# ucsdarclab/Python-SuPer

Measured on AMD Instinct MI355X. Metric: LM iterations/s (embedded-deformation LM, point-to-plane + ARAP + Rot), higher is better.
Workload: dtype f64

## Files before the change

### python-super_amd/csrc/slm_api.hip

```cpp
#include <atomic>
#include <condition_variable>
#include <functional>
#include <mutex>
#include <new>
#include <string>
#include <thread>
#include <algorithm>
#include <vector>
#include <cstdio>
#include <cstring>

#include "slm_common.h"
#include "slm_host.h"
#include "slm_launch.h"
#include "slm_prep.h"

static thread_local std::string g_err;
static const char* const kBadKnn =
    "slm_bind_frame: a KNN index (sf_knn_idx or ed_knn_idx) lies outside [0, J) or a surfel's row of sf_knn_idx repeats an id";

void slm_set_error_text(const char* msg) { g_err = msg; }

namespace {
template <typename T>
struct PinnedBuf {
  T* p = nullptr;
  size_t cap = 0, n = 0;
  hipError_t resize(size_t need) {
    if (need > cap) {
      if (p) (void)hipHostFree(p);
      p = nullptr;
      cap = 0;
      const size_t want = need + need / 8 + 16;
      const hipError_t e = hipHostMalloc((void**)&p, want * sizeof(T), hipHostMallocDefault);
      if (e != hipSuccess) return e;
      cap = want;
    }
    n = need;
    return hipSuccess;
  }
  void release() {
    if (p) (void)hipHostFree(p);
    p = nullptr;
    cap = n = 0;
  }
  T* data() { return p; }
  const T* data() const { return p; }
  size_t size() const { return n; }
  T* begin() { return p; }
  T* end() { return p + n; }
  T& operator[](size_t i) { return p[i]; }
  const T& operator[](size_t i) const { return p[i]; }
};

constexpr int kLossBlocks = 512;
constexpr int kRegBlocksMax = 64;

enum class DataForm {
  none,
  tuple,
  pairs,
  per_entry,
};
DataForm data_form_of(const slm_config& c, const slm_frame& f) {
  if (!c.use_data || f.N <= 0) return DataForm::none;
// ... 146 lines not shown

 private:
  void ensure(int n_workers) {
    while ((int)threads_.size() < n_workers) {
      const int id = (int)threads_.size();
      threads_.emplace_back([this, id] { loop(id); });
    }
  }
  void loop(int id) {
    int seen = 0;
    for (;;) {
      const std::function<void(int)>* job = nullptr;
      {
        std::unique_lock<std::mutex> lk(m_);
        cv_work_.wait(lk, [&] { return stop_ || generation_ != seen; });
        if (stop_) return;
        seen = generation_;
        if (id < n_active_) job = job_;
      }
      if (job) {
        (*job)(id + 1);
        std::lock_guard<std::mutex> lk(m_);
        if (--pending_ == 0) cv_done_.notify_all();
      }
    }
  }
  std::vector<std::thread> threads_;
  std::mutex m_;
  std::condition_variable cv_work_, cv_done_;
  const std::function<void(int)>* job_ = nullptr;
  int generation_ = 0, n_active_ = 0, pending_ = 0;
  bool stop_ = false;
};
}

struct slm_solver {
  PrepBuffers* prep = nullptr;
  BindPool bind_pool;
  AsyncWorker prep_worker;
  PrepBuffers* prep_async = nullptr;
  hipStream_t prep_stream = nullptr;
  std::vector<PrepBuffers*> bind_prep;
  std::vector<hipStream_t> bind_streams;
  std::vector<hipEvent_t> bind_events;
  std::mutex band_mutex;
  hipEvent_t drain_event = nullptr;
  double drain_est_ms = 0.0;
  int last_solver_form = -1;
  int last_dag_mode = -1;
  bool no_reuse = false;
  bool hybrid_batches = true;
  long dag_max_nodes = 8000;
  bool fuse_begin = true;
  bool pure_fill = true;
  bool profile = false;
  std::vector<hipEvent_t> ev_pool;
  std::vector<std::vector<hipEvent_t>> ev_runs;
  slm_config cfg{};
  std::vector<Slot> slots;
  FrameDev* frames_dev = nullptr;
  int* bw_dev = nullptr;
  int* bw_host = nullptr;
  int* reuse_dev = nullptr;
  int rank = 0, world = 1;
  bool shard_mode = false;
};
namespace {
bool solve_is_task_graph(const slm_solver* s, int n, int J);
}

static std::atomic<long long> g_reallocs{0}, g_realloc_bytes{0}, g_plan_builds{0}, g_plan_reuses{0}, g_plan_fill_hits{0};

template <typename T>
static hipError_t grow(T*& p, size_t& cap, size_t need) {
  if (need <= cap) return hipSuccess;
  const size_t want = need + need / 8;
  ++g_reallocs;
  g_realloc_bytes += (long long)(want * sizeof(T));
  return grow(p, cap, need, want);
}
template <typename T>
static hipError_t grow(GP<T>& p, size_t& cap, size_t need) {
  T* q = p;
  const hipError_t e = grow(q, cap, need);
  p = q;
  return e;
}

static int check_slots(slm_solver* s, int first, int n);

extern "C" {

const char* slm_last_error(void) { return g_err.c_str(); }

int slm_debug_last_solver_form(slm_solver* s) { return s ? s->last_solver_form : -1; }
int slm_debug_last_dag_mode(slm_solver* s) { return s ? s->last_dag_mode : -1; }

int slm_debug_counters(int64_t out[4]) {
  if (!out) return fail(SLM_ERR_INVALID, "slm_debug_counters: null output");
  out[0] = g_reallocs;
  out[1] = g_realloc_bytes;
  out[2] = g_plan_builds;
  out[3] = g_plan_reuses;
  return SLM_OK;
}

// ... 103 lines not shown
             sizeof(slm_frame), sizeof(slm_gf_config), sizeof(slm_gf_frame), sizeof(slm_iter_record));
    return fail(SLM_ERR_INVALID, buf);
  }
  return SLM_OK;
}

int slm_device_count(void) {
  int n = 0;
  if (hipGetDeviceCount(&n) != hipSuccess) return 0;
  return n;
}

int slm_create(const slm_config* cfg, slm_solver** out) {
  if (!cfg || !out) return fail(SLM_ERR_INVALID, "slm_create: null argument");
  if (cfg->max_frames < 1 || cfg->num_iterations < 0 || !(cfg->v > 0.0))
    return fail(SLM_ERR_INVALID, "slm_create: bad config");
  if (cfg->solver_path < 0 || cfg->solver_path > 4) return fail(SLM_ERR_INVALID, "slm_create: solver_path must be 0..4");
  if (cfg->data_path < 0 || cfg->data_path > 2) return fail(SLM_ERR_INVALID, "slm_create: data_path must be 0..2");
  if (slm_device_count() < 1) return fail(SLM_ERR_NO_DEVICE, "slm_create: no HIP device visible");
  slm_solver* s = new (std::nothrow) slm_solver();
  if (!s) return fail(SLM_ERR_HIP, "slm_create: out of host memory");
  s->cfg = *cfg;
  try {
    s->slots.resize(cfg->max_frames);
  } catch (...) {
    delete s;
    return fail(SLM_ERR_HIP, "slm_create: out of host memory");
  }
  hipError_t e = hipMalloc((void**)&s->frames_dev, sizeof(FrameDev) * cfg->max_frames);
  if (e == hipSuccess) e = hipMemset(s->frames_dev, 0, sizeof(FrameDev) * cfg->max_frames);
  if (e == hipSuccess) e = hipMalloc((void**)&s->bw_dev, 2 * sizeof(int));
  if (e == hipSuccess) e = hipMalloc((void**)&s->reuse_dev, sizeof(int) * cfg->max_frames);
  if (e == hipSuccess) e = hipMemset(s->reuse_dev, 0, sizeof(int) * cfg->max_frames);
  if (e == hipSuccess) e = hipHostMalloc((void**)&s->bw_host, 2 * sizeof(int), hipHostMallocDefault);
  if (e == hipSuccess) {
    s->prep = prep_create();
    if (!s->prep) e = hipErrorOutOfMemory;
  }
  if (e != hipSuccess) {
    g_err = std::string("slm_create: ") + hipGetErrorString(e);
    slm_destroy(s);
    return SLM_ERR_HIP;
  }
  {
    int dev = 0;
    (void)hipGetDevice(&dev);
    (void)dag_device_setup(dev, nullptr);
  }
  if (const char* hb = getenv("SLM_HYBRID")) s->hybrid_batches = atoi(hb) != 0;
  if (const char* dm = getenv("SLM_DAG_MAX_NODES")) s->dag_max_nodes = atol(dm);
  if (const char* nr = getenv("SLM_NO_REUSE")) s->no_reuse = atoi(nr) != 0;
  if (const char* pf = getenv("SLM_PURE_FILL")) s->pure_fill = atoi(pf) != 0;
  if (const char* fb = getenv("SLM_FUSE_BEGIN")) s->fuse_begin = atoi(fb) != 0;
  *out = s;
  return SLM_OK;
}

int slm_destroy(slm_solver* s) {
  if (!s) return SLM_OK;
  s->prep_worker.shutdown();
  s->bind_pool.shutdown();
  for (Slot& sl : s->slots) {
    FrameDev& h = sl.h;
    if (h.beta) (void)hipFree(h.beta);
    if (h.delta) (void)hipFree(h.delta);
    if (h.rhs) (void)hipFree(h.rhs);
    if (sl.band) (void)hipFree(sl.band);
    if (sl.linv) (void)hipFree(sl.linv);
    if (h.loss_part) (void)hipFree(h.loss_part);
    if (h.st) (void)hipFree(h.st);
    if (h.rec) (void)hipFree(h.rec);
    if (h.node_pk) (void)hipFree(h.node_pk);
    if (h.tgt_pn) (void)hipFree(h.tgt_pn);
    if (h.tgt_px) (void)hipFree(h.tgt_px);
    if (h.ev_rc) (void)hipFree(h.ev_rc);
    plan_free(sl.plan);
    pairplan_free(sl.pplan);
    if (sl.h_pin) (void)hipHostFree(sl.h_pin);
    sl.h_pairs.release();
    sl.h_knn.release();
    sl.h_pts.release();
    sl.h_pts64.release();
    if (sl.d_fronts) (void)hipFree(sl.d_fronts);
    if (sl.d_items) (void)hipFree(sl.d_items);
    if (sl.d_tile_kind) (void)hipFree(sl.d_tile_kind);
    if (sl.d_zero_tiles) (void)hipFree(sl.d_zero_tiles);
    if (sl.d_ints) (void)hipFree(sl.d_ints);
    if (sl.d_dests) (void)hipFree(sl.d_dests);
    if (sl.d_cur_dests) (void)hipFree(sl.d_cur_dests);
    if (sl.ftiles) (void)hipFree(sl.ftiles);
    if (sl.fvec) (void)hipFree(sl.fvec);
    if (sl.flinv) (void)hipFree(sl.flinv);
    if (sl.fmail) (void)hipFree(sl.fmail);
    if (sl.pairbuf) (void)hipFree(sl.pairbuf);
    if (sl.d_dag_flags) (void)hipFree(sl.d_dag_flags);
    if (sl.d_dag_trace) (void)hipFree(sl.d_dag_trace);
    if (sl.prep_fork) (void)hipEventDestroy(sl.prep_fork);
    if (sl.prep_done) (void)hipEventDestroy(sl.prep_done);
  }
  prep_destroy(s->prep);
  prep_destroy(s->prep_async);
  if (s->prep_stream) (void)hipStreamDestroy(s->prep_stream);
  for (PrepBuffers* pb : s->bind_prep) prep_destroy(pb);
  for (hipStream_t q : s->bind_streams) (void)hipStreamDestroy(q);
  for (hipEvent_t e : s->bind_events) (void)hipEventDestroy(e);
  for (auto& evs : s->ev_runs)
// ... 599 lines not shown
        if (rc != SLM_OK) {
          rcs[w] = rc;
          errs[w] = g_err;
          return;
        }
      }
      if (hipEventRecord(s->bind_events[w], s->bind_streams[w]) != hipSuccess) rcs[w] = SLM_ERR_HIP;
    } catch (...) {
      rcs[w] = SLM_ERR_HIP;
      try { errs[w] = "slm_bind_frames: out of host memory in a bind worker"; } catch (...) {}
    }
  };
  try {
    s->bind_pool.run(W, work);
  } catch (...) {
    return fail(SLM_ERR_HIP, "slm_bind_frames: could not start the bind workers");
  }
  for (int w = 0; w < W; ++w)
    if (rcs[w] != SLM_OK) return fail(rcs[w], errs[w].c_str());
  if (bind_trace_threshold() >= 0.0 && bt_now() - bt1 > bind_trace_threshold())
    fprintf(stderr, "[slm bind trace] batch of %d: drained the stream at %.3f (waited %.3f ms), workers done %.3f ms later\n",
            n_frames, bt1, bt1 - bt0, bt_now() - bt1);
  for (int w = 0; w < W; ++w) HIPCHK(hipStreamWaitEvent(st, s->bind_events[w], 0));
  return SLM_OK;
}

}

static int check_slots(slm_solver* s, int first, int n) {
  if (!s) return fail(SLM_ERR_INVALID, "null solver");
  if (first < 0 || n < 1 || first + n > (int)s->slots.size())
    return fail(SLM_ERR_INVALID, "slot range out of bounds");
  for (int i = first; i < first + n; ++i) {
    join_prepare(s, i);
    if (!s->slots[i].h.bound) return fail(SLM_ERR_UNBOUND, "slot used before slm_bind_frame");
    if (s->slots[i].h.f.K != s->slots[first].h.f.K)
      return fail(SLM_ERR_UNSUPPORTED, "the frames of one batch must have the same num_neighbors");
  }
  return SLM_OK;
}

namespace {
struct BatchDims {
  int maxN = 0, maxJKe = 0, nt_max = 0, wb_cap = 0, n_reg_part = 0;
  int max_pos = 0, max_blocks = 0, maxP = 0;
  int K = 0;
  int gram_variants = 0;
  bool nd = true;
  DataForm form = DataForm::none;
  const int* reuse = nullptr;
  bool fused_begin = false;
  int* accept_reuse = nullptr;
  int accept_eval = 0;
  int max_tasks = 0;
  int hybrid_cut = -2, hybrid_levels = -1, max_top_tasks = 0;
  std::vector<NDLevelSched> sched;
};
BatchDims dims_of(slm_solver* s, int first, int n, bool band = false) {
  BatchDims d;
  bool all_v1 = true, all_vk = true;
  for (int i = first; i < first + n; ++i) {
    const FrameDev& h = s->slots[i].h;
    d.maxN = std::max(d.maxN, h.f.N);
    d.K = (d.K == 0 || d.K == h.f.K) ? h.f.K : -1;
    d.maxJKe = std::max(d.maxJKe, h.f.J * h.f.K_ED);
    d.nt_max = std::max(d.nt_max, h.nt);
    d.wb_cap = std::max(d.wb_cap, h.wb);
    d.max_pos = std::max(d.max_pos, h.n_pos);
    d.max_blocks = std::max(d.max_blocks, h.n_blocks);
    all_v1 = all_v1 && h.v1_ready;
    all_vk = all_vk && h.vk_ready;
    if (h.v1_ready) d.gram_variants |= h.v2_ready ? 1 : 2;
    d.nd = d.nd && h.nd_ready;
    d.max_tasks = std::max(d.max_tasks, h.nd_ready ? h.n_dag_tasks : 0);
    if (h.nd_ready) {
      const int cut = h.n_dag_top_tasks > 0 ? h.dag_cut_depth : -1;
      if (d.hybrid_cut == -2) { d.hybrid_cut = cut; d.hybrid_levels = h.n_levels; }
      else if (d.hybrid_cut != cut || d.hybrid_levels != h.n_levels) d.hybrid_cut = -1;
      d.max_top_tasks = std::max(d.max_top_tasks, h.n_dag_top_tasks);
    }
    d.maxP = std::max(d.maxP, h.P);
  }
  d.nd = d.nd && !band;
  const slm_config& c = s->cfg;
  d.form = all_v1 ? DataForm::tuple : (d.nd && all_vk) ? DataForm::pairs : c.use_data ? DataForm::per_entry : DataForm::none;
  const bool tuple = d.form == DataForm::tuple;
  if (d.nd && tuple && c.phase_test && !s->no_reuse) d.reuse = s->reuse_dev + first;
  d.fused_begin = d.nd && tuple && d.gram_variants == 1 && d.max_pos > 0 && s->fuse_begin;
  if (tuple && c.phase_test) d.accept_reuse = s->reuse_dev + first;
  d.accept_eval = tuple ? 1 : 0;
  if (d.nd) {
    for (int i = first; i < first + n; ++i) {
      const auto& sc = s->slots[i].cache.nd.sched;
      if (sc.size() > d.sched.size()) d.sched.resize(sc.size(), NDLevelSched{0, 0, 0, 0, 0, -2, 0, -2, 0, -2});
      for (size_t l = 0; l < sc.size(); ++l) {
        NDLevelSched& m = d.sched[l];
        if (m.first == -2) m.first = sc[l].first;
        else if (m.first != sc[l].first || m.n_fronts != sc[l].n_fronts) m.first = -1;
        m.n_fronts = std::max(m.n_fronts, sc[l].n_fronts);
        m.max_npt = std::max(m.max_npt, sc[l].max_npt);
        m.max_nt = std::max(m.max_nt, sc[l].max_nt);
        m.max_pairs = std::max(m.max_pairs, sc[l].max_pairs);
        m.max_n2p = std::max(m.max_n2p, sc[l].max_n2p);
        if (m.schur_at == -2) m.schur_at = sc[l].schur_at;
        else if (m.schur_at != sc[l].schur_at || m.n_schur != sc[l].n_schur) m.schur_at = -1;
        m.n_schur = std::max(m.n_schur, sc[l].n_schur);
        if (m.pull_at == -2) m.pull_at = sc[l].pull_at;
        else if (m.pull_at != sc[l].pull_at || m.n_pull != sc[l].n_pull) m.pull_at = -1;
        m.n_pull = std::max(m.n_pull, sc[l].n_pull);
      }
    }
  }
  if (d.nd && n > 1) {
    for (int i = first; i < first + n; ++i)
      for (size_t l = s->slots[i].cache.nd.sched.size(); l < d.sched.size(); ++l)
        d.sched[l].first = d.sched[l].schur_at = d.sched[l].pull_at = -1;
  }
  for (auto& m : d.sched) {
    if (m.first == -2) m.first = -1;
    if (m.first < 0) m.schur_at = m.pull_at = -1;
    if (m.schur_at == -2) m.schur_at = -1;
    if (m.pull_at == -2) m.pull_at = -1;
  }
  if (s->cfg.use_arap || s->cfg.use_rot)
    d.n_reg_part = std::min(kRegBlocksMax, (d.maxJKe + 255) / 256);
  return d;
}

static bool solve_is_task_graph(const slm_solver* s, int n, int J) {
  return s->cfg.solver_path == 2 || (s->cfg.solver_path == 0 && (n <= 2 || (long)n * J <= s->dag_max_nodes));
}
static bool solve_is_hybrid(const slm_solver* s, int n, const BatchDims& d) {
  return !solve_is_task_graph(s, n, d.maxP / 7) && (s->cfg.solver_path == 4 || (s->cfg.solver_path == 0 && s->hybrid_batches)) &&
         d.hybrid_cut >= 0 && d.hybrid_levels == (int)d.sched.size() && d.hybrid_cut + 1 < d.hybrid_levels;
}
static int dag_cut_of(const slm_solver* s, int n, const BatchDims& d) {
  if (solve_is_task_graph(s, n, d.maxP / 7)) return -1;
  return solve_is_hybrid(s, n, d) ? d.hybrid_cut : -2;
}
int enqueue_front_solve(slm_solver* s, const FrameDev* fr, int n, const BatchDims& d, double u_override, hipStream_t st,
                        bool dag_reset_done = false, bool dag_check_later = false) {
  const bool dag = solve_is_task_graph(s, n, d.maxP / 7);
  const bool hybrid = solve_is_hybrid(s, n, d);
// ... 1 lines not shown
  int mode = -1;
  if (dag) {
    mode = launch_front_solve_dag(fr, n, d.max_tasks, u_override, st, -1, !dag_reset_done, !dag_check_later);
  } else if (hybrid) {
    const int n_levels = (int)d.sched.size(), l_cut = n_levels - 1 - d.hybrid_cut;
    launch_front_levels(fr, n, d.sched.data(), n_levels, l_cut, 0, u_override, st);
    mode = launch_front_solve_dag(fr, n, d.max_top_tasks, u_override, st, d.hybrid_cut, !dag_reset_done, !dag_check_later);
  } else {
    launch_front_solve(fr, n, d.sched.data(), (int)d.sched.size(), u_override, st);
  }
  s->last_dag_mode = mode;
  return mode;
}

void enqueue_zero(const FrameDev* fr, int n, const BatchDims& d, hipStream_t st, const int* reuse, int dag_cut, bool fused) {
  if (!d.nd) launch_iter_begin(fr, n, st);
  else if (!fused) launch_iter_begin_nd(fr, n, st, reuse, dag_cut);
}

void enqueue_jacobian(slm_solver* s, const FrameDev* fr, int n, const BatchDims& d, hipStream_t st, int eval_mode,
                      const int* reuse, int dag_cut, bool fused) {
  const double w = s->cfg.w_data;
  switch (d.form) {
    case DataForm::tuple:
      if (eval_mode >= 0) launch_data_eval(fr, n, kLossBlocks, w, eval_mode, st, reuse);
      if (fused) launch_begin_and_gram(fr, n, d.max_pos, w, st, reuse, dag_cut);
      else launch_data_gram(fr, n, d.max_pos, w, d.gram_variants, st, reuse);
      break;
    case DataForm::pairs: launch_data_grad_pairs(fr, n, d.maxN, d.K, w, st); break;
    case DataForm::per_entry: launch_data_grad(fr, n, d.maxN, d.K, w, st); break;
    case DataForm::none: break;
  }
}

enum class Shard { whole, before_exchange, after_exchange };
void enqueue_scatter(slm_solver* s, const FrameDev* fr, int n, const BatchDims& d, hipStream_t st, Shard part) {
  const slm_config& c = s->cfg;
  const bool tuple = d.form == DataForm::tuple;
  if (part == Shard::before_exchange) {
    if (tuple) launch_pair_reduce(fr, n, d.max_blocks, st);
    return;
  }
  if (part == Shard::after_exchange || d.form == DataForm::pairs) launch_pair_scatter(fr, n, d.max_blocks, st);
  else if (tuple && d.nd) launch_front_assemble(fr, n, d.max_blocks, st);
  else if (tuple) launch_band_assemble(fr, n, d.max_blocks, st);
  if (d.nd) {
    launch_reg_grad_nd(fr, n, d.maxP / 7, c.use_arap, c.w_arap, c.use_rot, c.w_rot, st);
    if (!c.use_arap && !c.use_rot) launch_front_load_rhs(fr, n, d.maxP, st);
  } else {
    launch_reg_grad(fr, n, d.maxJKe, c.use_arap, c.w_arap, c.use_rot, c.w_rot, st);
  }
}

void enqueue_data_loss(slm_solver* s, const FrameDev* fr, int n, const BatchDims& d, hipStream_t st, bool at_beta) {
  if (d.form == DataForm::tuple && !at_beta) launch_data_eval(fr, n, kLossBlocks, s->cfg.w_data, 0, st);
  else if (d.form != DataForm::none) launch_data_loss(fr, n, kLossBlocks, d.K, s->cfg.w_data, at_beta ? 0 : 1, st);
}
}

extern "C" {

static hipEvent_t take_event(slm_solver* s) {
  if (!s->ev_pool.empty()) {
    hipEvent_t e = s->ev_pool.back();
    s->ev_pool.pop_back();
    return e;
  }
  hipEvent_t e = nullptr;
  if (hipEventCreate(&e) != hipSuccess) return nullptr;
  return e;
}

int slm_set_shard(slm_solver* s, int32_t rank, int32_t world) {
  if (!s || world < 1 || rank < 0 || rank >= world) return fail(SLM_ERR_INVALID, "slm_set_shard: bad rank/world");
  if (s->cfg.data_path != 0 || s->cfg.solver_path == 1)
    return fail(SLM_ERR_UNSUPPORTED, "slm_set_shard: needs data_path 0 and a nested-dissection solver_path (0, 2, 3 or 4)");
  s->rank = rank;
  s->world = world;
  s->shard_mode = true;
  for (size_t i = 0; i < s->slots.size(); ++i) {
    join_prepare(s, (int)i);
    s->slots[i].model_ready = false;
    s->slots[i].h.bound = 0;
  }
  HIPCHK(hipMemset(s->frames_dev, 0, sizeof(FrameDev) * s->slots.size()));
  return SLM_OK;
}

static int shard_dims(slm_solver* s, int n_frames, BatchDims& d) {
  int rc = check_slots(s, 0, n_frames);
  if (rc) return rc;
  d = dims_of(s, 0, n_frames);
  if (!d.nd || (d.form != DataForm::tuple && d.form != DataForm::pairs))
    return fail(SLM_ERR_UNSUPPORTED, "sharded LM step: every slot needs a multifrontal data path (tuple-sorted or K-generic) and the ND solver");
  return SLM_OK;
}

int slm_lm_grad_local(slm_solver* s, int32_t n_frames, void* stream) {
  BatchDims d;
  int rc = shard_dims(s, n_frames, d);
  if (rc) return rc;
  hipStream_t st = (hipStream_t)stream;
  const FrameDev* fr = s->frames_dev;
  enqueue_zero(fr, n_frames, d, st, d.reuse, -2, false);
  enqueue_jacobian(s, fr, n_frames, d, st, 1, d.reuse, -2, false);
  enqueue_scatter(s, fr, n_frames, d, st, Shard::before_exchange);
  HIPCHK(hipGetLastError());
  return SLM_OK;
// ... 70 lines not shown
}

int slm_lm_exchange_get(slm_solver* s, int32_t slot, int32_t what, double* out, void* stream) {
  double* p;
  int64_t n;
  int rc = exchange_buf(s, slot, what, &p, &n);
  if (rc) return rc;
  if (!out) return fail(SLM_ERR_INVALID, "slm_lm_exchange_get: null output");
  HIPCHK(hipMemcpyAsync(out, p, sizeof(double) * n, hipMemcpyDeviceToDevice, (hipStream_t)stream));
  return SLM_OK;
}

int slm_lm_exchange_set(slm_solver* s, int32_t slot, int32_t what, const double* in, void* stream) {
  double* p;
  int64_t n;
  int rc = exchange_buf(s, slot, what, &p, &n);
  if (rc) return rc;
  if (!in) return fail(SLM_ERR_INVALID, "slm_lm_exchange_set: null input");
  HIPCHK(hipMemcpyAsync(p, in, sizeof(double) * n, hipMemcpyDeviceToDevice, (hipStream_t)stream));
  return SLM_OK;
}

static void enqueue_lm_iteration(slm_solver* s, int first, int n, const BatchDims& d, hipStream_t st, bool first_iteration) {
  const FrameDev* fr = s->frames_dev + first;
  const slm_config& c = s->cfg;
  std::vector<hipEvent_t>* evs = nullptr;
  if (s->profile) {
    s->ev_runs.emplace_back();
    evs = &s->ev_runs.back();
  }
  auto mark = [&]() {
    if (!evs) return;
    hipEvent_t e = take_event(s);
    if (e) (void)hipEventRecord(e, st);
    evs->push_back(e);
  };
  mark();
  const int dag_cut = d.nd ? dag_cut_of(s, n, d) : -2;
  enqueue_zero(fr, n, d, st, d.reuse, dag_cut, d.fused_begin);
  mark();
  const int eval_mode = (first_iteration || (c.phase_test && !d.reuse)) ? 1 : -1;
  enqueue_jacobian(s, fr, n, d, st, eval_mode, d.reuse, dag_cut, d.fused_begin);
  mark();
  enqueue_scatter(s, fr, n, d, st, Shard::whole);
  mark();
  const bool tail = c.use_data || d.n_reg_part > 0;
  int dag_mode = -1;
  if (d.nd) dag_mode = enqueue_front_solve(s, fr, n, d, -1.0, st, true, tail);
  else launch_band_solve(fr, n, d.nt_max, d.wb_cap, -1.0, st);
  if (tail)
    launch_after_solve(fr, n, c.use_data ? d.maxP / 7 : 0, d.n_reg_part, c.use_arap, c.w_arap, c.use_rot, c.w_rot,
                       dag_cut >= -1 ? ((dag_mode > 0 && (dag_mode & 1)) ? 2 : 1) : 0, st);
  mark();
  enqueue_data_loss(s, fr, n, d, st, false);
  mark();
  launch_accept(fr, n, c.phase_test, d.n_reg_part, std::max(c.num_iterations, 1), st, d.accept_reuse, d.accept_eval);
  mark();
}

int slm_run(slm_solver* s, int32_t n_frames, void* stream) {
  int rc = check_slots(s, 0, n_frames);
  if (rc) return rc;
  if (s->world > 1)
    return fail(SLM_ERR_UNSUPPORTED,
                "slm_run: the frame is sharded; drive slm_lm_grad_local / slm_lm_solve / slm_lm_loss_local / "
                "slm_lm_accept with the exchanges between them");
  hipStream_t st = (hipStream_t)stream;
  const slm_config& c = s->cfg;
  BatchDims d = dims_of(s, 0, n_frames);
  if (!d.nd) {
    std::lock_guard<std::mutex> lock(s->band_mutex);
    for (int i = 0; i < n_frames; ++i) {
      rc = ensure_band(s, i, st);
      if (rc) return rc;
    }
    d = dims_of(s, 0, n_frames);
  }
  for (int it = 0; it < c.num_iterations; ++it) enqueue_lm_iteration(s, 0, n_frames, d, st, it == 0);
  if (!d.accept_reuse) HIPCHK(hipMemsetAsync(s->reuse_dev, 0, sizeof(int) * n_frames, st));
  HIPCHK(hipGetLastError());
  return SLM_OK;
}

int slm_get_plan_info(slm_solver* s, int32_t slot, double* out_caller, int32_t capacity) {
  int rc = check_slots(s, slot, 1);
  if (rc) return rc;
  if (!out_caller || capacity < 0) return fail(SLM_ERR_INVALID, "slm_get_plan_info: bad output");
  const Slot& sl = s->slots[slot];
  const FrameDev& h = sl.h;
  double out[SLM_PLAN_INFO_DOUBLES];
  for (int i = 0; i < SLM_PLAN_INFO_DOUBLES; ++i) out[i] = 0.0;
  if (h.nd_ready) {
    out[0] = 0.0;
    out[1] = (double)sl.cache.nd.fronts.size();
    out[2] = (double)sl.cache.nd.level_start.size() - 1.0;
    out[3] = sl.cache.nd.flops;
    out[10] = sl.cache.nd.flops_exact;
    out[11] = (double)sl.cache.nd.dag_tasks.size() / 2.0;
    out[4] = 8.0 * (double)sl.cache.nd.tile_doubles;
    out[12] = (double)sl.n_piv_tiles;
    out[13] = (double)sl.n_pure_tiles;
  } else {
    out[0] = 1.0;
    const double w = (double)h.wb * SLM_NB;
    out[3] = (double)h.P * w * w;
    out[4] = 8.0 * (double)h.nt * (h.wb + 1) * SLM_NB * SLM_NB;
  }
  out[5] = h.n_tuples;
  out[6] = h.n_runs;
// ... 288 lines not shown
```

### python-super_amd/csrc/slm_data_v1.hip

```cpp
#include <cstdlib>

#include "slm_data.h"
#include "slm_begin.h"
#include "slm_launch.h"

#define ROW_STRIDE 17

__global__ void __launch_bounds__(256) k_data_eval(const FrameDev* __restrict__ frames, double lam, int mode,
                                                    const int* __restrict__ reuse) {
  __shared__ double sm[16];
  __shared__ int s_skip;
  if (mode == 1 && reuse && reuse[blockIdx.y]) return;
  const FrameDev& fd = frames[blockIdx.y];
  if (!fd.bound || !fd.v1_ready || fd.st->stopped) return;
  if (mode == 1) {
    if (threadIdx.x == 0) s_skip = __hip_atomic_load(&fd.st->eval_valid, __ATOMIC_RELAXED, __HIP_MEMORY_SCOPE_AGENT) == 1;
    __syncthreads();
    if (s_skip) return;
  }
  const double* npk = mode == 0 ? fd.node_pk_try.get() : fd.node_pk.get();
  const int p0 = 256 * fd.wg_lo, p1 = min(fd.n_pos, 256 * fd.wg_hi);
  double acc = 0.0;
  int cnt = 0;
  for (int pos = p0 + blockIdx.x * blockDim.x + threadIdx.x; pos < p1; pos += gridDim.x * blockDim.x) {
    const int4 ids = *reinterpret_cast<const int4*>(fd.s_idx + 4 * (size_t)pos);
    double2 o0 = make_double2(0.0, 0.0), o1 = make_double2(0.0, 0.0);
    if (ids.x >= 0) {
      double wk[4];
      ld_state4(fd.s_w, (size_t)pos, fd.f.state_f64, wk);
      const d3 pp = ld_state3(fd.s_pts, (size_t)pos, fd.f.state_f64);
      SurfelEval ev;
      eval_surfel_core<2, true>(fd, pp, ids, wk, lam, npk, ev);
      if (ev.match) {
        acc += ev.r * ev.r;
        ++cnt;
        o0 = make_double2(ev.r, ev.c[0]);
        o1 = make_double2(ev.c[1], ev.c[2]);
      }
    }
    double2* out = reinterpret_cast<double2*>(fd.ev_rc.get() + 4 * (size_t)pos);
    out[0] = o0;
    out[1] = o1;
  }
  const double s = block_sum(acc, sm);
  const double c = block_sum((double)cnt, sm);
  if (threadIdx.x == 0) {
    fd.loss_part[2 * blockIdx.x] = s;
    fd.loss_part[2 * blockIdx.x + 1] = c;
    LMState* st = fd.st;
    const unsigned long long old = __hip_atomic_fetch_add(&st->eval_acc, (1ull << 32) | (unsigned long long)(unsigned)(int)c,
                                                          __ATOMIC_RELAXED, __HIP_MEMORY_SCOPE_AGENT);
    if ((int)(old >> 32) == (int)gridDim.x - 1) {
      st->m_eval = (int)(unsigned)(old & 0xFFFFFFFFull) + (int)c;
      __hip_atomic_store(&st->eval_acc, 0ull, __ATOMIC_RELAXED, __HIP_MEMORY_SCOPE_AGENT);
      if (mode != 0) __hip_atomic_store(&st->eval_valid, 1, __ATOMIC_RELAXED, __HIP_MEMORY_SCOPE_AGENT);
    }
  }
}

template <bool MERGE, bool BEGIN = false>
__global__ void __launch_bounds__(256, 2) k_data_gram(const FrameDev* __restrict__ frames, double lam,
                                                       int dbg, const int* __restrict__ reuse, int n_gram = 0, int n_begin = 0,
                                                       int dag_cut = -2) {
  if (BEGIN && (int)blockIdx.x >= n_gram) {
    iter_begin_nd_body(frames[blockIdx.y], (int)blockIdx.x - n_gram, n_begin, reuse && reuse[blockIdx.y], dag_cut,
                       frames[blockIdx.y].v1_ready && frames[blockIdx.y].v2_ready);
    return;
  }
  __shared__ double rows[4][64 * ROW_STRIDE];
  __shared__ double recs[MERGE ? SLM_LB_MAX * SLM_WREC : 1];
  __shared__ uint8_t lidx[4][MERGE ? 160 : 4];
  if (reuse && reuse[blockIdx.y]) return;
  const FrameDev& fd = frames[blockIdx.y];
  if (!fd.bound || !fd.v1_ready) return;
  if (MERGE != (fd.v2_ready != 0)) return;
  const int w = threadIdx.x >> 6, l = threadIdx.x & 63;
  const int base = (blockIdx.x * 4 + w) * 64;
  if (blockIdx.x * 256 >= fd.n_pos) return;
  if (blockIdx.x == 0 && threadIdx.x == 0) fd.st->m_grad = fd.st->m_eval;
  if ((int)blockIdx.x < fd.wg_lo || (int)blockIdx.x >= fd.wg_hi) return;
  const bool wact = base < fd.n_pos;
  const int pos = base + l;
  const int lc = l & 15, lq = l >> 4;
  int rec0 = 0, nrec = 0;
  if (MERGE) {
    rec0 = fd.wg_first[blockIdx.x];
    nrec = fd.wg_last[blockIdx.x] - rec0 + 1;
  }
  int my_run = -1;
  int4 ids = {-1, -1, -1, -1};
  double wk[4] = {0, 0, 0, 0};
  d3 pp = {0, 0, 0};
  double2 e0 = make_double2(0.0, 0.0), e1 = make_double2(0.0, 0.0);
  if (wact) {
    my_run = fd.grp_run[(base >> 2) + lc];
    const double2* e2 = reinterpret_cast<const double2*>(fd.ev_rc.get() + 4 * (size_t)pos);
    e0 = e2[0];
    e1 = e2[1];
    ids = *reinterpret_cast<const int4*>(fd.s_idx + 4 * (size_t)pos);
    ld_state4(fd.s_w, (size_t)pos, fd.f.state_f64, wk);
    pp = ld_state3(fd.s_pts, (size_t)pos, fd.f.state_f64);
  }
  uint8_t lv0 = 0, lv1 = 0, lv2 = 0;
  if (MERGE && wact) {
#pragma unroll
    for (int k = 0; k < 3; ++k) {
      const int idx = l + 64 * k;
      const int g = idx / 10, e = idx - 10 * g;
      const int run = __shfl(my_run, g < 16 ? g : 0, 64);
      const uint8_t v = (idx < 160 && run >= 0) ? fd.run_lidx[10 * (size_t)run + e] : (uint8_t)0;
// ... 135 lines not shown
  const FrameDev& fd = frames[blockIdx.y];
  if (!fd.bound || !fd.v1_ready || fd.st->stopped) return;
  const int bi = blockIdx.x * 4 + (threadIdx.x >> 6);
  if (bi >= fd.n_blocks) return;
  const int l = threadIdx.x & 63;
  const unsigned key = (unsigned)fd.blk_key[bi];
  const int a = (int)(key / (unsigned)fd.f.J), b = (int)(key % (unsigned)fd.f.J);
  const int ca = l / 7, cb = l % 7;
  const bool act = (l < 49) && (a != b || ca >= cb);
  const bool jt = (a == b) && l >= 49 && l < 56;
  double acc = 0.0;
  if (fd.v2_ready) {
    const int s0 = fd.blk2_start[bi], s1 = fd.blk2_start[bi + 1];
    if (l < SLM_WREC)
      for (int s = s0; s < s1; ++s) acc += fd.wgslab[(size_t)fd.blk2_entry[s] * SLM_WREC + l];
  } else {
    const int s0 = fd.blk_start[bi], s1 = fd.blk_start[bi + 1];
    for (int s = s0; s < s1; ++s) {
      const int pl = fd.blk_entry[s];
      const int run = pl >> 4, pa = (pl >> 2) & 3, pb = pl & 3;
      const double* G = fd.slab + (size_t)run * SLM_SLAB_STRIDE;
      if (act) acc += gram_at(G, 7 * pa + ca, 7 * pb + cb);
      else if (jt) acc += gram_at(G, 28, 7 * pa + (l - 49));
    }
  }
  if (act) *band_entry(fd, 7 * a + ca, 7 * b + cb) = acc;
  else if (jt) fd.rhs[7 * a + (l - 49)] = -acc;
}

void launch_begin_and_gram(const FrameDev* frames_dev, int n_frames, int max_pos, double lam, hipStream_t st, const int* reuse,
                           int dag_cut) {
  int dbg = 0;
#ifdef SLM_STAMPS
  if (const char* e = getenv("SLM_DBG")) dbg = atoi(e);
#endif
  const int n_gram = (max_pos + 255) / 256, n_begin = 1024;
  hipLaunchKernelGGL((k_data_gram<true, true>), dim3(n_gram + n_begin, n_frames), dim3(256), 0, st, frames_dev, lam, dbg, reuse, n_gram,
                     n_begin, dag_cut);
}

void launch_data_gram(const FrameDev* frames_dev, int n_frames, int max_pos, double lam, int variants,
                      hipStream_t st, const int* reuse) {
  if (max_pos <= 0) return;
  int dbg = 0;
#ifdef SLM_STAMPS
  if (const char* e = getenv("SLM_DBG")) dbg = atoi(e);
#endif
  const dim3 grid((max_pos + 255) / 256, n_frames);
  if (variants & 1) hipLaunchKernelGGL(k_data_gram<true>, grid, dim3(256), 0, st, frames_dev, lam, dbg, reuse);
  if (variants & 2) hipLaunchKernelGGL(k_data_gram<false>, grid, dim3(256), 0, st, frames_dev, lam, dbg, reuse);
}

void launch_data_eval(const FrameDev* frames_dev, int n_frames, int n_blocks, double lam, int mode, hipStream_t st,
                      const int* reuse) {
  hipLaunchKernelGGL(k_data_eval, dim3(n_blocks, n_frames), dim3(256), 0, st, frames_dev, lam, mode, reuse);
}

void launch_band_assemble(const FrameDev* frames_dev, int n_frames, int max_blocks, hipStream_t st) {
  if (max_blocks <= 0) return;
  hipLaunchKernelGGL(k_band_assemble, dim3((max_blocks + 3) / 4, n_frames), dim3(256), 0, st, frames_dev);
}
```

### python-super_amd/csrc/slm_launch.h

```cpp
#pragma once
#include "slm_common.h"

void launch_data_grad(const FrameDev*, int, int, int, double, hipStream_t);
void launch_data_grad_pairs(const FrameDev*, int, int, int, double, hipStream_t);
void launch_data_loss(const FrameDev*, int, int, int, double, int, hipStream_t);
void launch_data_resid(const FrameDev*, int, int, int, double, double*, uint8_t*, int32_t*, hipStream_t);

void launch_data_gram(const FrameDev*, int, int, double, int, hipStream_t, const int* reuse = nullptr);
void launch_begin_and_gram(const FrameDev*, int, int, double, hipStream_t, const int* reuse, int dag_cut);
void launch_data_eval(const FrameDev*, int, int, double, int mode, hipStream_t, const int* reuse = nullptr);
void launch_band_assemble(const FrameDev*, int, int, hipStream_t);

void launch_front_assemble(const FrameDev*, int, int, hipStream_t);
void launch_pair_reduce(const FrameDev*, int, int, hipStream_t);
void launch_pair_scatter(const FrameDev*, int, int, hipStream_t);
void launch_reg_grad_nd(const FrameDev*, int, int, int, double, int, double, hipStream_t);
void launch_front_load_rhs(const FrameDev*, int, int, hipStream_t);
void launch_iter_begin_nd(const FrameDev*, int, hipStream_t, const int* reuse, int dag_cut);
void launch_front_solve(const FrameDev*, int, const NDLevelSched*, int, double, hipStream_t);
void launch_front_levels(const FrameDev*, int, const NDLevelSched*, int, int, int, double, hipStream_t);

int launch_front_solve_dag(const FrameDev*, int, int, double, hipStream_t, int cut, bool reset, bool check);
int dag_device_setup(int dev, int* xcd8_out);
int dag_last_mode();
hipError_t set_dag_timeout_ticks(long long);
void launch_dag_abort_check(const FrameDev*, int, hipStream_t);

void launch_bandwidth(const slm_frame&, int*, hipStream_t);
void launch_band_solve(const FrameDev*, int, int, int, double, hipStream_t);
void launch_band_to_dense(const FrameDev*, int, double*, hipStream_t);
void launch_dense_to_band(const FrameDev*, const double*, const double*, hipStream_t);

void launch_reg_grad(const FrameDev*, int, int, int, double, int, double, hipStream_t);
void launch_after_solve(const FrameDev*, int, int, int, int, double, int, double, int, hipStream_t);
void launch_reg_loss(const FrameDev*, int, int, int, double, int, double, int, hipStream_t);

void launch_init_slot(const FrameDev*, int, int, const slm_config&, hipStream_t);
void launch_iter_begin(const FrameDev*, int, hipStream_t);
void launch_pack_nodes(const FrameDev*, int, int, hipStream_t);
void launch_make_trial(const FrameDev*, int, int, hipStream_t);
void launch_pack_target(int, const float*, const float*, float4*, hipStream_t);
void launch_pack_target_px(int, const int*, const uint8_t*, const float*, const float*, float4*, hipStream_t);
void launch_accept(const FrameDev*, int, int, int, int, hipStream_t, int* reuse = nullptr, int eval_pass = 0);
void launch_loss_out(const FrameDev*, int, int, double*, hipStream_t);
void launch_zero_reg_part(const FrameDev*, int, int, hipStream_t);
void launch_update(int, int, int, float*, float*, const int*, const float*, float*, float*, const double*, hipStream_t);
void launch_update64(int, int, int, double*, double*, const int*, const double*, double*, double*, const double*,
                     hipStream_t);
void launch_knn(int, int, int, int, const float*, const float*, int*, float*, hipStream_t);
void launch_knn64(int, int, int, int, const double*, const double*, const int*, const int*, int*, double*, int*,
                  hipStream_t);
void launch_knn_weights64(int, int, int, const int*, const double*, const double*, int, const double*, const double*,
                          double*, uint8_t*, hipStream_t);
void launch_knn_weights(int, int, int, const int*, const float*, const float*, float*, uint8_t*, hipStream_t);
```

### python-super_amd/csrc/slm_misc.hip

```cpp
#include "slm_common.h"
#include "slm_launch.h"

__global__ void __launch_bounds__(256) k_init_slot(const FrameDev* __restrict__ frames, int slot,
                                                    double u0, double v, double minimal_loss0,
                                                    int num_iterations) {
  const FrameDev& fd = frames[slot];
  const int t = blockIdx.x * blockDim.x + threadIdx.x;
  if (t < fd.f.J) {
    double* b = fd.beta + 7 * t;
    b[0] = 1.0;
#pragma unroll
    for (int c = 1; c < 7; ++c) b[c] = 0.0;
    const double ident[7] = {1.0, 0.0, 0.0, 0.0, 0.0, 0.0, 0.0};
    pack_node(fd.node_pk + (size_t)SLM_NPK * t, ident, ld_state3(frame_in(fd).ed_points, (size_t)t, fd.f.state_f64));
  }
  if (t < num_iterations) {
    slm_iter_record r;
    r.loss = 0.0;
    r.u = 0.0;
    r.accepted = 0;
    r.status = SLM_ITER_NOT_RUN;
    r.M_grad = 0;
    r.M_loss = 0;
    fd.rec[t] = r;
  }
  if (t == 0) {
    LMState s;
    s.u = u0;
    s.v = v;
    s.minimal_loss = minimal_loss0;
    s.iter = 0;
    s.stopped = 0;
    s.m_grad = 0;
    s.m_loss = 0;
    s.chol_fail = 0;
    s.m_grad_local = 0;
    s.eval_valid = 0;
    s.m_eval = 0;
    s.eval_acc = 0;
    *fd.st = s;
  }
}

__global__ void __launch_bounds__(256) k_iter_begin(const FrameDev* __restrict__ frames) {
  const FrameDev& fd = frames[blockIdx.y];
  if (!fd.bound || fd.st->stopped) return;
  const size_t nband = (size_t)fd.nt * (fd.wb + 1) * SLM_NB * SLM_NB;
  const size_t nrhs = (size_t)fd.nt * SLM_NB;
  double2* b2 = reinterpret_cast<double2*>(fd.band.get());
  for (size_t e = (size_t)blockIdx.x * blockDim.x + threadIdx.x; e < nband / 2;
       e += (size_t)gridDim.x * blockDim.x)
    b2[e] = make_double2(0.0, 0.0);
  for (size_t e = (size_t)blockIdx.x * blockDim.x + threadIdx.x; e < nrhs;
       e += (size_t)gridDim.x * blockDim.x)
    fd.rhs[e] = 0.0;
  if (blockIdx.x == 0 && threadIdx.x == 0) {
    fd.st->m_grad = 0;
    fd.st->chol_fail = 0;
  }
}

__global__ void __launch_bounds__(1024) k_accept(const FrameDev* __restrict__ frames, int phase_test,
                                                  int n_reg_part, int n_rec, int* __restrict__ reuse, int eval_pass) {
  __shared__ double sm[16];
  __shared__ int s_accept;
  const FrameDev& fd = frames[blockIdx.y];
  if (!fd.bound) return;
  LMState* st = fd.st;
  if (st->stopped) return;
  const int it = st->iter;
  if (st->chol_fail) {
    if (threadIdx.x == 0) {
      if (it < n_rec) {
        slm_iter_record r = fd.rec[it];
        r.status = st->chol_fail == 2 ? SLM_ITER_SOLVER_TIMEOUT : SLM_ITER_SOLVER_FAILED;
        r.u = st->u;
        r.M_grad = st->m_grad;
        fd.rec[it] = r;
      }
      st->stopped = 1;
    }
    return;
  }
  double ls = 0.0, cnt = 0.0;
  for (int b = threadIdx.x; b < fd.n_loss_part; b += blockDim.x) {
    ls += fd.loss_part[2 * b];
    cnt += fd.loss_part[2 * b + 1];
  }
  const double* reg = fd.loss_part + 2 * (size_t)fd.n_loss_part;
  for (int b = threadIdx.x; b < n_reg_part; b += blockDim.x) ls += reg[2 * b] + reg[2 * b + 1];
  const double loss = block_sum(ls, sm);
  const double m = block_sum(cnt, sm);
  if (threadIdx.x == 0) {
    int acc = 1;
    const double u_used = st->u;
    if (phase_test) {
      if (loss < st->minimal_loss) {
        st->minimal_loss = loss;
        st->u = u_used / st->v;
      } else {
        acc = 0;
        st->u = u_used * st->v;
      }
    }
    slm_iter_record r;
    r.loss = loss;
    r.u = u_used;
    r.accepted = acc;
    r.status = SLM_ITER_OK;
    r.M_grad = st->m_grad;
    r.M_loss = (int)m;
    if (it < n_rec) fd.rec[it] = r;
    st->iter = it + 1;
    s_accept = acc;
    if (reuse) reuse[blockIdx.y] = acc ? 0 : 1;
    st->eval_valid = eval_pass ? acc : 0;
  }
  __syncthreads();
  if (s_accept) {
    for (int e = threadIdx.x; e < fd.P; e += blockDim.x) {
      const double b = fd.beta[e] + fd.delta[e];
      fd.beta[e] = b;
      fd.node_pk[(size_t)SLM_NPK * (e / 7) + e % 7] = b;
    }
  }
}

__global__ void __launch_bounds__(256) k_pack_nodes(const FrameDev* __restrict__ frames, int slot) {
  const FrameDev& fd = frames[slot];
  const int j = blockIdx.x * blockDim.x + threadIdx.x;
  if (j >= fd.f.J) return;
  double bb[7];
#pragma unroll
  for (int c = 0; c < 7; ++c) bb[c] = fd.beta[7 * j + c];
  pack_node(fd.node_pk + (size_t)SLM_NPK * j, bb, ld_state3(frame_in(fd).ed_points, (size_t)j, fd.f.state_f64));
}

__global__ void __launch_bounds__(256) k_make_trial(const FrameDev* __restrict__ frames) {
  const FrameDev& fd = frames[blockIdx.y];
  if (!fd.bound || fd.st->stopped) return;
  const int j = blockIdx.x * blockDim.x + threadIdx.x;
  if (j >= fd.f.J) return;
  double bb[7];
#pragma unroll
  for (int c = 0; c < 7; ++c) bb[c] = fd.beta[7 * j + c] + fd.delta[7 * j + c];
  pack_node(fd.node_pk_try + (size_t)SLM_NPK * j, bb, ld_state3(frame_in(fd).ed_points, (size_t)j, fd.f.state_f64));
}

__global__ void __launch_bounds__(256) k_pack_target(int T, const float* __restrict__ pts,
                                                      const float* __restrict__ nrm,
                                                      float4* __restrict__ out) {
  const int t = blockIdx.x * blockDim.x + threadIdx.x;
  if (t >= T) return;
  out[2 * (size_t)t] = make_float4(pts[3 * t], pts[3 * t + 1], pts[3 * t + 2], 0.f);
  out[2 * (size_t)t + 1] = make_float4(nrm[3 * t], nrm[3 * t + 1], nrm[3 * t + 2], 0.f);
}

__global__ void __launch_bounds__(256) k_pack_target_px(int HW, const int* __restrict__ index_map, const uint8_t* __restrict__ valid,
                                                         const float* __restrict__ pts, const float* __restrict__ nrm,
                                                         float4* __restrict__ out) {
  const int p = blockIdx.x * blockDim.x + threadIdx.x;
  if (p >= HW) return;
  const int t = index_map[p];
  float4 a = make_float4(0.f, 0.f, 0.f, 0.f), b = make_float4(0.f, 0.f, 0.f, valid[p] ? 1.f : 0.f);
  if (t >= 0) {
    a = make_float4(pts[3 * (size_t)t], pts[3 * (size_t)t + 1], pts[3 * (size_t)t + 2], 1.f);
    b = make_float4(nrm[3 * (size_t)t], nrm[3 * (size_t)t + 1], nrm[3 * (size_t)t + 2], b.w);
  }
  out[2 * (size_t)p] = a;
  out[2 * (size_t)p + 1] = b;
}

__global__ void __launch_bounds__(256) k_loss_out(const FrameDev* __restrict__ frames, int slot,
                                                   int n_reg_part, double* __restrict__ out) {
  __shared__ double sm[16];
  const FrameDev& fd = frames[slot];
  double d = 0.0, c = 0.0, a = 0.0, r = 0.0;
  for (int b = threadIdx.x; b < fd.n_loss_part; b += blockDim.x) {
// ... 367 lines not shown
```

Baseline: 3327.

## Fuse LM accept step into data-eval kernel via last-block-done pattern

New measurement: 3298. About the same (-0.9%).

```diff
diff --git a/python-super_amd/csrc/slm_accept.h b/python-super_amd/csrc/slm_accept.h
--- /dev/null
+++ b/python-super_amd/csrc/slm_accept.h
@@ -0,0 +1,88 @@
+#pragma once
+#include "slm_common.h"
+
+struct AcceptArgs {
+  int on, phase_test, n_reg_part, n_rec, eval_pass;
+  int* reuse;
+};
+
+template <bool FRESH>
+__device__ __forceinline__ void accept_body(const FrameDev& fd, int slot, int phase_test, int n_reg_part, int n_rec,
+                                            int* __restrict__ reuse, int eval_pass, double* sm, int* s_accept) {
+  if (!fd.bound) return;
+  LMState* st = fd.st;
+  if (st->stopped) return;
+  const int it = st->iter;
+  if (st->chol_fail) {
+    if (threadIdx.x == 0) {
+      if (it < n_rec) {
+        slm_iter_record r = fd.rec[it];
+        r.status = st->chol_fail == 2 ? SLM_ITER_SOLVER_TIMEOUT : SLM_ITER_SOLVER_FAILED;
+        r.u = st->u;
+        r.M_grad = st->m_grad;
+        fd.rec[it] = r;
+      }
+      st->stopped = 1;
+    }
+    return;
+  }
+  const int nw = (int)blockDim.x >> 6, lane = threadIdx.x & 63, wv = threadIdx.x >> 6;
+  const double* reg = fd.loss_part + 2 * (size_t)fd.n_loss_part;
+  for (int v = 0; v * (int)blockDim.x < 1024; ++v) {
+    const int vt = v * (int)blockDim.x + (int)threadIdx.x;
+    double ls = 0.0, cnt = 0.0;
+    for (int b = vt; b < fd.n_loss_part; b += 1024) {
+      if (FRESH) {
+        ls += __hip_atomic_load(fd.loss_part.get() + 2 * b, __ATOMIC_RELAXED, __HIP_MEMORY_SCOPE_AGENT);
+        cnt += __hip_atomic_load(fd.loss_part.get() + 2 * b + 1, __ATOMIC_RELAXED, __HIP_MEMORY_SCOPE_AGENT);
+      } else {
+        ls += fd.loss_part[2 * b];
+        cnt += fd.loss_part[2 * b + 1];
+      }
+    }
+    for (int b = vt; b < n_reg_part; b += 1024) ls += reg[2 * b] + reg[2 * b + 1];
+    ls = wave_sum(ls);
+    cnt = wave_sum(cnt);
+    if (lane == 0) {
+      sm[v * nw + wv] = ls;
+      sm[16 + v * nw + wv] = cnt;
+    }
+  }
+  __syncthreads();
+  if (threadIdx.x == 0) {
+    double loss = 0.0, m = 0.0;
+    for (int i = 0; i < 16; ++i) loss += sm[i];
+    for (int i = 0; i < 16; ++i) m += sm[16 + i];
+    int acc = 1;
+    const double u_used = st->u;
+    if (phase_test) {
+      if (loss < st->minimal_loss) {
+        st->minimal_loss = loss;
+        st->u = u_used / st->v;
+      } else {
+        acc = 0;
+        st->u = u_used * st->v;
+      }
+    }
+    slm_iter_record r;
+    r.loss = loss;
+    r.u = u_used;
+    r.accepted = acc;
+    r.status = SLM_ITER_OK;
+    r.M_grad = st->m_grad;
+    r.M_loss = (int)m;
+    if (it < n_rec) fd.rec[it] = r;
+    st->iter = it + 1;
+    *s_accept = acc;
+    if (reuse) reuse[slot] = acc ? 0 : 1;
+    st->eval_valid = eval_pass ? acc : 0;
+  }
+  __syncthreads();
+  if (*s_accept) {
+    for (int e = threadIdx.x; e < fd.P; e += blockDim.x) {
+      const double b = fd.beta[e] + fd.delta[e];
+      fd.beta[e] = b;
+      fd.node_pk[(size_t)SLM_NPK * (e / 7) + e % 7] = b;
+    }
+  }
+}
diff --git a/python-super_amd/csrc/slm_api.hip b/python-super_amd/csrc/slm_api.hip
--- a/python-super_amd/csrc/slm_api.hip
+++ b/python-super_amd/csrc/slm_api.hip
@@ -11,6 +11,7 @@
 #include <cstring>
 
 #include "slm_common.h"
+#include "slm_accept.h"
 #include "slm_host.h"
 #include "slm_launch.h"
 #include "slm_prep.h"
@@ -263,6 +264,7 @@
   bool hybrid_batches = true;
   long dag_max_nodes = 8000;
   bool fuse_begin = true;
+  bool fuse_shell = true;
   bool pure_fill = true;
   bool profile = false;
   std::vector<hipEvent_t> ev_pool;
@@ -472,6 +474,7 @@
   if (const char* nr = getenv("SLM_NO_REUSE")) s->no_reuse = atoi(nr) != 0;
   if (const char* pf = getenv("SLM_PURE_FILL")) s->pure_fill = atoi(pf) != 0;
   if (const char* fb = getenv("SLM_FUSE_BEGIN")) s->fuse_begin = atoi(fb) != 0;
+  if (const char* fs = getenv("SLM_FUSE_SHELL")) s->fuse_shell = atoi(fs) != 0;
   *out = s;
   return SLM_OK;
 }
@@ -1177,6 +1180,7 @@
   bool fused_begin = false;
   int* accept_reuse = nullptr;
   int accept_eval = 0;
+  bool fused_accept = false;
   int max_tasks = 0;
   int hybrid_cut = -2, hybrid_levels = -1, max_top_tasks = 0;
   std::vector<NDLevelSched> sched;
@@ -1214,6 +1218,7 @@
   d.fused_begin = d.nd && tuple && d.gram_variants == 1 && d.max_pos > 0 && s->fuse_begin;
   if (tuple && c.phase_test) d.accept_reuse = s->reuse_dev + first;
   d.accept_eval = tuple ? 1 : 0;
+  d.fused_accept = d.nd && tuple && c.use_data && s->world <= 1 && s->fuse_shell && (!c.phase_test || d.reuse);
   if (d.nd) {
     for (int i = first; i < first + n; ++i) {
       const auto& sc = s->slots[i].cache.nd.sched;
@@ -1321,8 +1326,9 @@
   }
 }
 
-void enqueue_data_loss(slm_solver* s, const FrameDev* fr, int n, const BatchDims& d, hipStream_t st, bool at_beta) {
-  if (d.form == DataForm::tuple && !at_beta) launch_data_eval(fr, n, kLossBlocks, s->cfg.w_data, 0, st);
+void enqueue_data_loss(slm_solver* s, const FrameDev* fr, int n, const BatchDims& d, hipStream_t st, bool at_beta,
+                       const AcceptArgs* accept = nullptr) {
+  if (d.form == DataForm::tuple && !at_beta) launch_data_eval(fr, n, kLossBlocks, s->cfg.w_data, 0, st, nullptr, accept);
   else if (d.form != DataForm::none) launch_data_loss(fr, n, kLossBlocks, d.K, s->cfg.w_data, at_beta ? 0 : 1, st);
 }
 }
@@ -1499,9 +1505,10 @@
     launch_after_solve(fr, n, c.use_data ? d.maxP / 7 : 0, d.n_reg_part, c.use_arap, c.w_arap, c.use_rot, c.w_rot,
                        dag_cut >= -1 ? ((dag_mode > 0 && (dag_mode & 1)) ? 2 : 1) : 0, st);
   mark();
-  enqueue_data_loss(s, fr, n, d, st, false);
+  const AcceptArgs ac = {1, c.phase_test, d.n_reg_part, std::max(c.num_iterations, 1), d.accept_eval, d.accept_reuse};
+  enqueue_data_loss(s, fr, n, d, st, false, d.fused_accept ? &ac : nullptr);
   mark();
-  launch_accept(fr, n, c.phase_test, d.n_reg_part, std::max(c.num_iterations, 1), st, d.accept_reuse, d.accept_eval);
+  if (!d.fused_accept) launch_accept(fr, n, ac.phase_test, ac.n_reg_part, ac.n_rec, st, ac.reuse, ac.eval_pass);
   mark();
 }
 
diff --git a/python-super_amd/csrc/slm_data_v1.hip b/python-super_amd/csrc/slm_data_v1.hip
--- a/python-super_amd/csrc/slm_data_v1.hip
+++ b/python-super_amd/csrc/slm_data_v1.hip
@@ -2,13 +2,14 @@
 
 #include "slm_data.h"
 #include "slm_begin.h"
+#include "slm_accept.h"
 #include "slm_launch.h"
 
 #define ROW_STRIDE 17
 
 __global__ void __launch_bounds__(256) k_data_eval(const FrameDev* __restrict__ frames, double lam, int mode,
-                                                    const int* __restrict__ reuse) {
-  __shared__ double sm[16];
+                                                    const int* __restrict__ reuse, AcceptArgs ac) {
+  __shared__ double sm[32];
   __shared__ int s_skip;
   if (mode == 1 && reuse && reuse[blockIdx.y]) return;
   const FrameDev& fd = frames[blockIdx.y];
@@ -45,8 +46,15 @@
   const double s = block_sum(acc, sm);
   const double c = block_sum((double)cnt, sm);
   if (threadIdx.x == 0) {
-    fd.loss_part[2 * blockIdx.x] = s;
-    fd.loss_part[2 * blockIdx.x + 1] = c;
+    if (ac.on) {
+      __hip_atomic_store(fd.loss_part.get() + 2 * blockIdx.x, s, __ATOMIC_RELAXED, __HIP_MEMORY_SCOPE_AGENT);
+      __hip_atomic_store(fd.loss_part.get() + 2 * blockIdx.x + 1, c, __ATOMIC_RELAXED, __HIP_MEMORY_SCOPE_AGENT);
+      asm volatile("s_waitcnt vmcnt(0)" ::: "memory");
+      s_skip = 0;
+    } else {
+      fd.loss_part[2 * blockIdx.x] = s;
+      fd.loss_part[2 * blockIdx.x + 1] = c;
+    }
     LMState* st = fd.st;
     const unsigned long long old = __hip_atomic_fetch_add(&st->eval_acc, (1ull << 32) | (unsigned long long)(unsigned)(int)c,
                                                           __ATOMIC_RELAXED, __HIP_MEMORY_SCOPE_AGENT);
@@ -54,8 +62,17 @@
       st->m_eval = (int)(unsigned)(old & 0xFFFFFFFFull) + (int)c;
       __hip_atomic_store(&st->eval_acc, 0ull, __ATOMIC_RELAXED, __HIP_MEMORY_SCOPE_AGENT);
       if (mode != 0) __hip_atomic_store(&st->eval_valid, 1, __ATOMIC_RELAXED, __HIP_MEMORY_SCOPE_AGENT);
-    }
-  }
+      if (ac.on) {
+        s_skip = 1;
+        __builtin_amdgcn_fence(__ATOMIC_ACQUIRE, "agent");
+        asm volatile("s_waitcnt vmcnt(0)" ::: "memory");
+      }
+    }
+  }
+  if (!ac.on) return;
+  __syncthreads();
+  if (!s_skip) return;
+  accept_body<true>(fd, blockIdx.y, ac.phase_test, ac.n_reg_part, ac.n_rec, ac.reuse, ac.eval_pass, sm, &s_skip);
 }
 
 template <bool MERGE, bool BEGIN = false>
@@ -297,8 +314,10 @@
 }
 
 void launch_data_eval(const FrameDev* frames_dev, int n_frames, int n_blocks, double lam, int mode, hipStream_t st,
-                      const int* reuse) {
-  hipLaunchKernelGGL(k_data_eval, dim3(n_blocks, n_frames), dim3(256), 0, st, frames_dev, lam, mode, reuse);
+                      const int* reuse, const AcceptArgs* accept) {
+  AcceptArgs ac = {0, 0, 0, 0, 0, nullptr};
+  if (accept && mode == 0) ac = *accept;
+  hipLaunchKernelGGL(k_data_eval, dim3(n_blocks, n_frames), dim3(256), 0, st, frames_dev, lam, mode, reuse, ac);
 }
 
 void launch_band_assemble(const FrameDev* frames_dev, int n_frames, int max_blocks, hipStream_t st) {
diff --git a/python-super_amd/csrc/slm_launch.h b/python-super_amd/csrc/slm_launch.h
--- a/python-super_amd/csrc/slm_launch.h
+++ b/python-super_amd/csrc/slm_launch.h
@@ -8,7 +8,9 @@
 
 void launch_data_gram(const FrameDev*, int, int, double, int, hipStream_t, const int* reuse = nullptr);
 void launch_begin_and_gram(const FrameDev*, int, int, double, hipStream_t, const int* reuse, int dag_cut);
-void launch_data_eval(const FrameDev*, int, int, double, int mode, hipStream_t, const int* reuse = nullptr);
+struct AcceptArgs;
+void launch_data_eval(const FrameDev*, int, int, double, int mode, hipStream_t, const int* reuse = nullptr,
+                      const AcceptArgs* accept = nullptr);
 void launch_band_assemble(const FrameDev*, int, int, hipStream_t);
 
 void launch_front_assemble(const FrameDev*, int, int, hipStream_t);
diff --git a/python-super_amd/csrc/slm_misc.hip b/python-super_amd/csrc/slm_misc.hip
--- a/python-super_amd/csrc/slm_misc.hip
+++ b/python-super_amd/csrc/slm_misc.hip
@@ -1,4 +1,5 @@
 #include "slm_common.h"
+#include "slm_accept.h"
 #include "slm_launch.h"
 
 __global__ void __launch_bounds__(256) k_init_slot(const FrameDev* __restrict__ frames, int slot,
@@ -62,68 +63,9 @@
 
 __global__ void __launch_bounds__(1024) k_accept(const FrameDev* __restrict__ frames, int phase_test,
                                                   int n_reg_part, int n_rec, int* __restrict__ reuse, int eval_pass) {
-  __shared__ double sm[16];
+  __shared__ double sm[32];
   __shared__ int s_accept;
-  const FrameDev& fd = frames[blockIdx.y];
-  if (!fd.bound) return;
-  LMState* st = fd.st;
-  if (st->stopped) return;
-  const int it = st->iter;
-  if (st->chol_fail) {
-    if (threadIdx.x == 0) {
-      if (it < n_rec) {
-        slm_iter_record r = fd.rec[it];
-        r.status = st->chol_fail == 2 ? SLM_ITER_SOLVER_TIMEOUT : SLM_ITER_SOLVER_FAILED;
-        r.u = st->u;
-        r.M_grad = st->m_grad;
-        fd.rec[it] = r;
-      }
-      st->stopped = 1;
-    }
-    return;
-  }
-  double ls = 0.0, cnt = 0.0;
-  for (int b = threadIdx.x; b < fd.n_loss_part; b += blockDim.x) {
-    ls += fd.loss_part[2 * b];
-    cnt += fd.loss_part[2 * b + 1];
-  }
-  const double* reg = fd.loss_part + 2 * (size_t)fd.n_loss_part;
-  for (int b = threadIdx.x; b < n_reg_part; b += blockDim.x) ls += reg[2 * b] + reg[2 * b + 1];
-  const double loss = block_sum(ls, sm);
-  const double m = block_sum(cnt, sm);
-  if (threadIdx.x == 0) {
-    int acc = 1;
-    const double u_used = st->u;
-    if (phase_test) {
-      if (loss < st->minimal_loss) {
-        st->minimal_loss = loss;
-        st->u = u_used / st->v;
-      } else {
-        acc = 0;
-        st->u = u_used * st->v;
-      }
-    }
-    slm_iter_record r;
-    r.loss = loss;
-    r.u = u_used;
-    r.accepted = acc;
-    r.status = SLM_ITER_OK;
-    r.M_grad = st->m_grad;
-    r.M_loss = (int)m;
-    if (it < n_rec) fd.rec[it] = r;
-    st->iter = it + 1;
-    s_accept = acc;
-    if (reuse) reuse[blockIdx.y] = acc ? 0 : 1;
-    st->eval_valid = eval_pass ? acc : 0;
-  }
-  __syncthreads();
-  if (s_accept) {
-    for (int e = threadIdx.x; e < fd.P; e += blockDim.x) {
-      const double b = fd.beta[e] + fd.delta[e];
-      fd.beta[e] = b;
-      fd.node_pk[(size_t)SLM_NPK * (e / 7) + e % 7] = b;
-    }
-  }
+  accept_body<false>(frames[blockIdx.y], blockIdx.y, phase_test, n_reg_part, n_rec, reuse, eval_pass, sm, &s_accept);
 }
 
 __global__ void __launch_bounds__(256) k_pack_nodes(const FrameDev* __restrict__ frames, int slot) {
```
